# apple/ml-fastvlm

Hardware: AMD Instinct MI355X
Metric: images/sec FastViTHD encode_images @1024x1024 bf16 (higher is better)
Workload: dtype bf16; 1 GPU; BASELINE.json configs[1]: FastViTHD encoder + mlp2x_gelu projector (H=896), batch=32/GPU synthetic 1024x1024 bf16 images in [0,1), seeded synthetic weights, single GPU; global_batch=32, image_size=1024, parallelism=dp1, hip_graph=False, attention_operands=bf16, ffn_precision=auto (calibrated on the benchmark batch), range guard on

## Files before the change

### include/fvhd.h

```cpp
#ifndef FVHD_H
#define FVHD_H

#include <stddef.h>
#include <stdint.h>

#ifdef __cplusplus
extern "C" {
#endif

typedef struct fvhd_ctx fvhd_ctx;
typedef void* fvhd_stream_t;

#define FVHD_F32 0
#define FVHD_F16 1
#define FVHD_BF16 2

#define FVHD_EPI_NONE 0
#define FVHD_EPI_BIAS 1
#define FVHD_EPI_BIAS_GELU 2
#define FVHD_EPI_BIAS_LS_RESID 3

#define FVHD_VERSION 510
int fvhd_version(void);
const char* fvhd_last_error(void);
// ... 57 lines not shown
int fvhd_op_dw3_dw7(fvhd_stream_t stream, const void* x, void* y, void* a, const float* w3, const float* b3, const float* w7,
                    const float* b7, int B, int H, int W, int C, void* amax_bits);
int fvhd_dw3_dw7_supported(int B, int H, int W, int C, int force);
int fvhd_dw7s2_mfma_supported(int B, int H, int W, int Cin, int force);
int fvhd_op_dw7s2_mfma(fvhd_stream_t stream, const void* x, void* y, const float* w, const float* bias, int B, int H, int W, int Cin);
#define FVHD_AMAX_SLOTS 64
int fvhd_op_dw7_amax(fvhd_stream_t stream, const void* x, void* y, const float* w, const float* bias, int B, int H, int W, int C, int mfma,
                     void* amax_bits);
int fvhd_op_gemm(fvhd_stream_t stream, const void* A, const void* Wt, const float* bias, const float* ls,
                 const void* resid, void* out, int M, int N, int K, int epilogue, int out_dtype);
int fvhd_op_gemm_splitk_ls(fvhd_stream_t stream, const void* A, const void* Wt, const float* bias, const float* ls, const void* resid, void* out,
                           float* partial, int M, int N, int K, int splits);
int fvhd_gemm_splitk_plan(int M, int N, int K);
#define FVHD_GEMM_PLAN_V1_NF4_BK64 0
#define FVHD_GEMM_PLAN_V1_NF4_BK32 1
#define FVHD_GEMM_PLAN_V1_NF3_BK64 2
#define FVHD_GEMM_PLAN_V1_NF3_BK32 3
#define FVHD_GEMM_PLAN_V1S 4
#define FVHD_GEMM_PLAN_256X128 5
#define FVHD_GEMM_PLAN_256X256 6
#define FVHD_GEMM_PLAN_PINGPONG 7
#define FVHD_GEMM_PLAN_128X192 8
int fvhd_gemm_kernel_plan(int M, int N, int K, int epilogue, int out_dtype);
int fvhd_op_layernorm(fvhd_stream_t stream, const void* x, void* y, const float* w, const float* b, int M, int C, float eps);
int fvhd_op_attention(fvhd_stream_t stream, const void* qkv, void* out, int B, int N, int C);
int fvhd_op_attention_fp8(fvhd_stream_t stream, const void* qkv, void* out, int B, int N, int C);
int fvhd_op_stem_conv(fvhd_stream_t stream, const void* img, int dtype, void* out, const float* w, const float* bias, int B, int R);
int fvhd_op_stem_fused(fvhd_stream_t stream, const void* img, int dtype, void* out, const float* w0, const float* b0,
                       const float* w1, const float* b1, const void* w2, const float* b2, int B, int R);
int fvhd_op_se_head(fvhd_stream_t stream, const void* y, float* pooled, float* scale, const float* wr, const float* br,
                    const float* we, const float* be, void* out, int out_dtype, int B, int T, int C, int RD);

int fvhd_ffn_fused_supported(int C);
int fvhd_ffn_pack(int C, const float* host_fc1, const float* host_fc2, void* host_w1img, void* host_w2img, int precision);
int fvhd_op_ffn_fused(fvhd_stream_t stream, const void* A, const void* w1img, const float* b1, const void* w2img,
                      const float* b2, const float* ls, void* X, int M, int C, int precision);

int fvhd_op_preprocess(fvhd_stream_t stream, const void* src, int src_h, int src_w, int64_t src_pitch, int pad_top, int pad_left,
                       uint32_t bg, const int32_t* hbounds, const int32_t* hcoef, int hk, const int32_t* vbounds, const int32_t* vcoef,
                       int vk, int row0, int nrows, void* tmp, const float* lut, int R, void* out, int out_dtype);

int fvhd_op_splice(fvhd_stream_t stream, const int64_t* ids, const int32_t* start, const int32_t* seqlen, const int64_t* feat_row0,
                   const int64_t* labels_in, const void* table, const void* feats, void* out, uint8_t* mask_out, int64_t* pos_out,
                   int64_t* labels_out, int B, int L, int H, int max_len, int64_t vocab, int64_t n_feat_rows, int left_pad, int dtype);

#define FVHD_EPI_RESID 4
// ... 148 lines not shown
```

### ml_fastvlm_amd/_lib.py

```python
from __future__ import annotations

import ctypes as C
import os
from typing import Dict, Tuple

_HERE = os.path.dirname(os.path.abspath(__file__))
LIB_PATH = os.environ.get("FVHD_LIB") or os.path.join(_HERE, "libfvhd.so")

ABI_VERSION = 501
SAMPLING_VERSION = 502
WIDE_BATCH_VERSION = 503
W8_VERSION = 504
BEAM_VERSION = 505
PROCESSORS_VERSION = 506
LOOKUP_VERSION = 507
GEMM_PLAN_VERSION = 508
EXTEND_VERSION = 509
(GEMM_PLAN_V1_NF4_BK64, GEMM_PLAN_V1_NF4_BK32, GEMM_PLAN_V1_NF3_BK64, GEMM_PLAN_V1_NF3_BK32, GEMM_PLAN_V1S, GEMM_PLAN_256X128, GEMM_PLAN_256X256,
 GEMM_PLAN_PINGPONG, GEMM_PLAN_128X192) = range(9)
MAX_DECODE_BATCH = 64
MAX_VERIFY_ROWS = 16
MAX_EOS_IDS, MAX_SUPPRESS_IDS = 16, 256
MAX_LOGPROBS = 16
W_BF16, W_E4M3 = 0, 1
# ... 140 lines not shown
            "fvhd_llm_cache_rewind": (ci, [vp, vp, vp]),
            "fvhd_op_attention_extend": (ci, [vp, vp, vp, vp, vp, vp, ci, ci, ci, ci, ci, ci, vp]),
            "fvhd_op_cache_append": (ci, [vp, vp, vp, vp, vp, vp, ci, ci, ci, ci, ci, ci, vp, vp]),
            "fvhd_op_extend_positions": (ci, [vp, vp, vp, vp, ci, ci]),
            "fvhd_op_cache_rewind": (ci, [vp, vp, ci, vp, vp, ci, vp, vp]),
        })
    if hasattr(lib, "fvhd_op_lm_score"):
        sig.update({
            "fvhd_lm_score_scratch_bytes": (C.c_size_t, [ci, ci, ci]),
            "fvhd_lm_score_plan": (ci, [ci, ci, ci]),
            "fvhd_op_lm_score": (ci, [vp, vp, vp, vp, ci, ci, ci, vp, vp, vp, C.c_size_t]),
            "fvhd_llm_score_reserve": (ci, [vp, ci]),
            "fvhd_llm_score": (ci, [vp, vp, vp, vp, vp]),
        })
    if hasattr(lib, "fvhd_op_dec_gemm_w4"):
        sig.update({
            "fvhd_llm_debug_packed_mxfp4": (ci, [vp, ci, ci, vp, vp, vp]),
            "fvhd_op_quantize_mxfp4": (ci, [vp, vp, ci, ci, vp, vp]),
            "fvhd_op_dec_gemm_w4": (ci, [vp, ci, vp, ci, vp, cf, vp, vp, ci, ci, vp, vp, vp, vp, ci]),
            "fvhd_op_dec_qkv_w4": (ci, [vp, vp, ci, ci, vp, cf, vp, vp, vp, vp, vp, vp, ci, cf, vp, vp, ci, vp, ci, ci, ci, vp, vp, ci]),
            "fvhd_op_dec_lm_argmax_w4": (ci, [vp, vp, ci, vp, cf, vp, vp, ci, ci, vp, vp, vp, vp]),
            "fvhd_op_w4_unpack": (ci, [vp, vp, vp, vp, ci, ci, ci]),
        })
    if hasattr(lib, "fvhd_op_dec_logprobs"):
        sig.update({
            "fvhd_dec_logprobs_scratch_bytes": (C.c_size_t, [ci, ci, ci]),
            "fvhd_op_dec_logprobs": (ci, [vp, vp, vp, ci, ci, ci, vp, vp, vp, vp, C.c_size_t]),
            "fvhd_llm_set_logprobs": (ci, [vp, ci]),
            "fvhd_llm_logprobs": (ci, [vp, vp, ci, vp, vp, vp, vp]),
        })
    del fp, cl
    for name, (res, args) in sig.items():
        fn = getattr(lib, name)
        fn.restype = res
        fn.argtypes = args


def load():
    global _lib
    if _lib is None:
        if not os.path.exists(LIB_PATH):
            raise FvhdError(
                f"{LIB_PATH} not found: the HIP extension is not built. Run `python -m ml_fastvlm_amd.build` "
                "(hipcc, gfx950). There is no CPU fallback for this path.")
        lib = C.CDLL(LIB_PATH)
        lib.fvhd_version.restype, lib.fvhd_version.argtypes = C.c_int, []
# ... 37 lines not shown
    lib = load()
    got = lib.fvhd_version()
    if got < PROCESSORS_VERSION:
        raise FvhdError(f"{LIB_PATH} reports ABI version {got}: logits processors (fvhd_llm_set_logits_processors, "
                        f"fvhd_op_dec_logits_process) need {PROCESSORS_VERSION} - rebuild the library (`python -m ml_fastvlm_amd.build`)")
    return lib


def lookup_lib():
    lib = load()
    got = lib.fvhd_version()
    if got < LOOKUP_VERSION:
        raise FvhdError(f"{LIB_PATH} reports ABI version {got}: prompt-lookup decoding (fvhd_llm_spec_reserve, fvhd_llm_verify, "
                        f"fvhd_llm_lookup_step, ...) needs {LOOKUP_VERSION} - rebuild the library (`python -m ml_fastvlm_amd.build`)")
    return lib


def gemm_plan_lib():
    lib = load()
    got = lib.fvhd_version()
    if got < GEMM_PLAN_VERSION:
        raise FvhdError(f"{LIB_PATH} reports ABI version {got}: the GEMM dispatch query (fvhd_gemm_kernel_plan) needs {GEMM_PLAN_VERSION} - "
                        "rebuild the library (`python -m ml_fastvlm_amd.build`)")
    return lib


def extend_lib():
    lib = load()
    got = lib.fvhd_version()
    if got < EXTEND_VERSION:
        raise FvhdError(f"{LIB_PATH} reports ABI version {got}: extending a started cache (fvhd_llm_extend, fvhd_llm_cache_rewind, "
                        f"fvhd_op_attention_extend, ...) needs {EXTEND_VERSION} - rebuild the library (`python -m ml_fastvlm_amd.build`)")
    return lib


def score_lib():
    lib = load()
    if not hasattr(lib, "fvhd_op_lm_score"):
        raise FvhdError(f"{LIB_PATH} (ABI version {lib.fvhd_version()}) was built before scoring (fvhd_llm_score, fvhd_llm_score_reserve, "
                        "fvhd_op_lm_score, ...) - rebuild the library (`python -m ml_fastvlm_amd.build`)")
    return lib


def w4_lib():
    lib = load()
    if not hasattr(lib, "fvhd_op_dec_gemm_w4"):
# ... 201 lines not shown
```

### ml_fastvlm_amd/csrc/fvhd_api.hip

```cpp
#include <hip/hip_runtime.h>
#include <stdint.h>
#include <stdlib.h>
#include <string.h>

#include <cmath>
#include <map>
#include <string>
#include <vector>

#include "api_host.h"
#include "launchers.h"

namespace {

thread_local std::string g_err;

int fail(const std::string& msg, int code = 1)
{
    g_err = msg;
    return code ? code : 1;
}

int hip_fail(const char* what, hipError_t e)
{
// ... 1151 lines not shown
    }
    return e ? hip_fail("fvhd_op_dw7_amax", (hipError_t)e) : 0;
}

int fvhd_op_gemm(fvhd_stream_t st, const void* A, const void* Wt, const float* bias, const float* ls, const void* resid,
                 void* out, int M, int N, int K, int epilogue, int out_dtype)
{
    if (!A || !Wt || !out) return fail("fvhd_op_gemm: NULL pointer");
    if ((epilogue == FVHD_EPI_BIAS || epilogue == FVHD_EPI_BIAS_GELU || epilogue == FVHD_EPI_BIAS_LS_RESID) && !bias) return fail("fvhd_op_gemm: this epilogue needs bias");
    if (epilogue == FVHD_EPI_BIAS_LS_RESID && !ls) return fail("fvhd_op_gemm: FVHD_EPI_BIAS_LS_RESID needs ls");
    if ((epilogue == FVHD_EPI_BIAS_LS_RESID || epilogue == FVHD_EPI_RESID) && !resid) return fail("fvhd_op_gemm: this epilogue needs resid");
    int e = fvhd_launch_gemm((hipStream_t)st, A, Wt, bias, ls, resid, out, M, N, K, epilogue, out_dtype);
    return e ? hip_fail("fvhd_op_gemm", (hipError_t)e) : 0;
}

int fvhd_op_gemm_splitk_ls(fvhd_stream_t st, const void* A, const void* Wt, const float* bias, const float* ls, const void* resid, void* out,
                           float* partial, int M, int N, int K, int splits)
{
    if (!A || !Wt || !bias || !ls || !resid || !out || !partial) return fail("fvhd_op_gemm_splitk_ls: NULL pointer");
    int e = fvhd_launch_gemm_splitk_ls((hipStream_t)st, A, Wt, bias, ls, resid, out, partial, M, N, K, splits);
    return e ? hip_fail("fvhd_op_gemm_splitk_ls", (hipError_t)e) : 0;
}

int fvhd_op_layernorm(fvhd_stream_t st, const void* x, void* y, const float* w, const float* b, int M, int C, float eps)
{
    int e = fvhd_launch_layernorm((hipStream_t)st, x, y, w, b, M, C, eps);
    return e ? hip_fail("fvhd_op_layernorm", (hipError_t)e) : 0;
}

int fvhd_op_attention(fvhd_stream_t st, const void* qkv, void* out, int B, int N, int C)
{
    int e = fvhd_launch_attention((hipStream_t)st, qkv, out, B, N, C, 0);
    return e ? hip_fail("fvhd_op_attention", (hipError_t)e) : 0;
}

int fvhd_op_attention_fp8(fvhd_stream_t st, const void* qkv, void* out, int B, int N, int C)
{
    int e = fvhd_launch_attention((hipStream_t)st, qkv, out, B, N, C, 1);
    return e ? hip_fail("fvhd_op_attention_fp8", (hipError_t)e) : 0;
}

int fvhd_op_stem_conv(fvhd_stream_t st, const void* img, int dtype, void* out, const float* w, const float* bias, int B, int R)
{
    int e = fvhd_launch_stem_conv((hipStream_t)st, img, dtype, out, w, bias, B, R);
    return e ? hip_fail("fvhd_op_stem_conv", (hipError_t)e) : 0;
}
// ... 88 lines not shown
```

### ml_fastvlm_amd/csrc/gemm.hip

```cpp
#include "fvhd_common.h"
#include "launchers.h"
#include "gemm_layout.h"
#include "rope.h"
#include <stdlib.h>

#define EPI_NONE 0
#define EPI_BIAS 1
#define EPI_BIAS_GELU 2
#define EPI_BIAS_LS_RESID 3
#define EPI_RESID 4
static_assert(FVHD_EPI_SWIGLU_ID == 5 && FVHD_ODT_BF16_ID == FVHD_BF16, "gemm_layout.h ids");
#define EPI_SWIGLU 5

#define EPI_BIAS_ROPE 6

struct RopeArgs {
    const long* pos; const float* table; bf16* kcache; bf16* vcache;
    int M, T, nh, nkv, P; float theta;
};

template <int BK>
FVHD_DEV int lds_off(int row, int ks)
{
    if constexpr (BK == 64) return row * 128 + ((ks ^ ((row >> 1) & 7)) << 4);
// ... 222 lines not shown
#pragma unroll
            for (int i = 0; i < W_CH; ++i) rw[i] = *(const u32x4*)(w_src[i] + ko);
        }
#pragma unroll
        for (int kk = 0; kk < BK / 32; ++kk) {
            bf16x8 af[MF], wf[NF];
            const int ks = kk * 4 + g;
#pragma unroll
            for (int i = 0; i < MF; ++i) af[i] = *(const bf16x8*)(ldsA + lds_off<BK>(wm * 64 + i * 16 + lr, ks));
#pragma unroll
            for (int j = 0; j < NF; ++j) wf[j] = *(const bf16x8*)(ldsW + lds_off<BK>(wn * 16 * NF + j * 16 + lr, ks));
#pragma unroll
            for (int i = 0; i < MF; ++i)
#pragma unroll
                for (int j = 0; j < NF; ++j)
                    acc[i][j] = __builtin_amdgcn_mfma_f32_16x16x32_bf16(wf[j], af[i], acc[i][j], 0, 0, 0);
        }
    }

    gemm_epilogue<MF, NF, EPI, ODT>(acc, bias, ls, resid, out, M, N, m0 + wm * 64, n0 + wn * 16 * NF, lr, g);
}

template <int BN, int BK = 64, int NWV = 8> struct G2Cfg {
    static constexpr int RS = BK == 64 ? (BN == 256 ? 2 : 3) : (NWV == 4 ? 3 : BN == 256 ? 4 : 6), STAGE = (256 + BN) * BK * 2, LDS = RS * STAGE;
};
template <int BK> FVHD_DEV int lds_swz(int row) { return BK == 64 ? ((row >> 1) & 7) : ((0 - (row >> 2)) & 3); }

FVHD_DEV void glds_piece(unsigned voff, const void* sbase, unsigned m0v)
{
    unsigned keep;
    asm volatile("s_mov_b32 %0, m0\n\ts_mov_b32 m0, %3\n\ts_nop 0\n\tglobal_load_lds_dwordx4 %1, %2\n\ts_mov_b32 m0, %0"
                 : "=&s"(keep) : "v"(voff), "s"(sbase), "s"(m0v) : "memory");
}

template <int EPI, int ODT, int NWV, int BN = 128, int BKT = 64, int ABL = 0>
__global__ __launch_bounds__(64 * NWV, (NWV == 4 && BKT == 32) ? 2 : 1) void gemm256_kernel(
    const bf16* __restrict__ A, const bf16* __restrict__ Wt, const float* __restrict__ bias,
    const float* __restrict__ ls, const bf16* resid, void* out, int M, int N, int K, int tiles_n, int nwg)
{
    constexpr int BM = 256, BK = BKT, WN = BN / 64, WM = NWV / WN, MF = BM / WM / 16, NF = 4, RS = G2Cfg<BN, BK, NWV>::RS, STAGE = G2Cfg<BN, BK, NWV>::STAGE;
    constexpr int RPP = 1024 / (BK * 2), LPR = BK / 8;
    constexpr int PA = (BM / RPP) / NWV, PW = (BN / RPP) / NWV;
    static_assert(WM * WN == NWV && MF * 16 * WM == BM, "wave grid");
    extern __shared__ __attribute__((aligned(16))) char lds2[];
    const int tid = threadIdx.x, lane = tid & 63, wave = __builtin_amdgcn_readfirstlane(tid >> 6);
    const int wm = wave / WN, wn = wave % WN;
    const int lr = lane & 15, g = lane >> 4;
    constexpr int GN = BN == 256 ? 4 : 8;
    const int tiles_m = nwg / tiles_n;
    auto tile_origin = [&](int t, int& m0_, int& n0_) {
        const int L = xcd_remap(t, nwg);
        const int grp = L / (tiles_m * GN), rem = L - grp * tiles_m * GN;
        const int wg = min(GN, tiles_n - grp * GN);
        const int tm = rem / wg, tn = grp * GN + (rem - tm * wg);
        m0_ = tm * BM; n0_ = tn * BN;
    };
    int tile = blockIdx.x, m0, n0;
    tile_origin(tile, m0, n0);

    constexpr int GRP = EpiGrp<NF, EPI, ODT>::value;
    static_assert(GRP == 1 || BK == 64, "the W row permutation is written for 8-row pieces");
    const int rip = lane / LPR;
    unsigned va[2], vw[2];
#pragma unroll
    for (int par = 0; par < 2; ++par) {
        const int sw = lds_swz<BK>(par * RPP + rip);
        va[par] = (unsigned)((rip * K + (((lane % LPR) ^ sw) * 8)) * 2);
        vw[par] = (unsigned)((wpiece_lane_row<GRP>(rip) * K + (((lane % LPR) ^ sw) * 8)) * 2);
    }
    const char* abase = (const char*)(A + (size_t)(m0 + wave * RPP * PA) * K);
    const char* wbase = (const char*)(Wt + (size_t)n0 * K);
// ... 24 lines not shown
        for (int j = 0; j < NF; ++j) acc[i][j] = f32x4{0.f, 0.f, 0.f, 0.f};

    for (int kt = 0; kt < nk; ++kt) {
        {
            const int later = nk - 1 - kt < RS - 2 ? nk - 1 - kt : RS - 2;
            if (later == RS - 2 && RS > 2) asm volatile("s_waitcnt vmcnt(%0)" :: "n"((RS - 2) * (PA + PW)) : "memory");
            else if (RS > 5 && later == 3) asm volatile("s_waitcnt vmcnt(%0)" :: "n"(3 * (PA + PW)) : "memory");
            else if (RS > 4 && later == 2) asm volatile("s_waitcnt vmcnt(%0)" :: "n"(2 * (PA + PW)) : "memory");
            else if (RS > 3 && later == 1) asm volatile("s_waitcnt vmcnt(%0)" :: "n"(1 * (PA + PW)) : "memory");
            else asm volatile("s_waitcnt vmcnt(0)" ::: "memory");
        }
        __syncthreads();
        if (kt + RS - 1 < nk) issue(kt + RS - 1);
        const char* ldsA = lds2 + (kt % RS) * STAGE;
        const char* ldsW = ldsA + BM * BK * 2;
        if constexpr (ABL == 2) continue;
#pragma unroll
        for (int kk = 0; kk < BK / 32; ++kk) {
            bf16x8 af[MF], wf[NF];
            const int ks = kk * 4 + g;
#pragma unroll
            for (int i = 0; i < MF; ++i) af[i] = *(const bf16x8*)(ldsA + lds_off<BK>(wm * 16 * MF + i * 16 + lr, ks));
#pragma unroll
            for (int j = 0; j < NF; ++j) wf[j] = *(const bf16x8*)(ldsW + lds_off<BK>(wn * 64 + j * 16 + lr, ks));
#pragma unroll
            for (int i = 0; i < MF; ++i)
#pragma unroll
                for (int j = 0; j < NF; ++j)
                    acc[i][j] = __builtin_amdgcn_mfma_f32_16x16x32_bf16(wf[j], af[i], acc[i][j], 0, 0, 0);
        }
    }
    const int em0 = m0 + wm * 16 * MF, en0 = n0 + wn * 64;
    tile += gridDim.x;
    const bool more = tile < nwg;
    if (more) {
        __syncthreads();
        tile_origin(tile, m0, n0);
        abase = (const char*)(A + (size_t)(m0 + wave * RPP * PA) * K);
        wbase = (const char*)(Wt + (size_t)n0 * K);
#pragma unroll
        for (int i = 0; i < RS - 1; ++i)
            if (i < nk) issue(i);
    }
    gemm_epilogue<MF, NF, EPI, ODT, true>(acc, bias, ls, resid, out, M, N, em0, en0, lr, g);
    if (!more) break;
  }
}

constexpr int kG128Stages = 4, kG128Stage = (128 + 128) * 64 * 2, kG128Lds = kG128Stages * kG128Stage;
template <int EPI, int ODT>
__global__ __launch_bounds__(256, 1) void gemm128s_kernel(
    const bf16* __restrict__ A, const bf16* __restrict__ Wt, const float* __restrict__ bias,
    const float* __restrict__ ls, const bf16* resid, void* out_, int M, int N, int K, int tiles_n, int nwg, int ldk, RopeArgs rope)
{
    constexpr int BM = 128, BK = 64, MF = 4, NF = 4, RS = kG128Stages, STAGE = kG128Stage, RPP = 8, PA = 4, PW = 4;
// ... 54 lines not shown
        __syncthreads();
        if (kt + RS - 1 < nk) issue(kt + RS - 1);
        const char* ldsA = lds2 + (kt % RS) * STAGE;
        const char* ldsW = ldsA + BM * BK * 2;
#pragma unroll
        for (int kk = 0; kk < BK / 32; ++kk) {
            bf16x8 af[MF], wf[NF];
            const int ks = kk * 4 + g;
#pragma unroll
            for (int i = 0; i < MF; ++i) af[i] = *(const bf16x8*)(ldsA + lds_off<BK>(wm * 64 + i * 16 + lr, ks));
#pragma unroll
            for (int j = 0; j < NF; ++j) wf[j] = *(const bf16x8*)(ldsW + lds_off<BK>(wn * 64 + j * 16 + lr, ks));
#pragma unroll
            for (int i = 0; i < MF; ++i)
#pragma unroll
                for (int j = 0; j < NF; ++j)
                    acc[i][j] = __builtin_amdgcn_mfma_f32_16x16x32_bf16(wf[j], af[i], acc[i][j], 0, 0, 0);
        }
    }
    if constexpr (EPI == EPI_BIAS_ROPE) gemm_epilogue_rope<MF>(acc, bias, (bf16*)out, rope, M, N, m0 + wm * 64, n0 + wn * 64, lr, g);
    else gemm_epilogue<MF, NF, EPI, ODT, true>(acc, bias, ls, resid, out, M, N, m0 + wm * 64, n0 + wn * 64, lr, g);
}

template <int EPI, int ODT>
__global__ __launch_bounds__(512) void gemm_pp_kernel(
    const bf16* __restrict__ A, const bf16* __restrict__ Wt, const float* __restrict__ bias,
    const float* __restrict__ ls, const bf16* resid, void* out, int M, int N, int K, int tiles_n, int nwg)
{
    constexpr int BM = 256, BN = 256, BK = 64, MF = 8, NF = 4, STAGE = (BM + BN) * 128;
    extern __shared__ __attribute__((aligned(16))) char lds2[];
    const int tid = threadIdx.x, lane = tid & 63, wave = __builtin_amdgcn_readfirstlane(tid >> 6);
    const int grp = wave >> 2, wn = wave & 3;
    const int lr = lane & 15, g = lane >> 4;
    const int L = xcd_remap(blockIdx.x, nwg);
    constexpr int GN = 4;
    const int tiles_m = nwg / tiles_n;
    const int sg = L / (tiles_m * GN), rem = L - sg * tiles_m * GN;
    const int wgw = min(GN, tiles_n - sg * GN);
    const int tm = rem / wgw, tn = sg * GN + (rem - tm * wgw);
    const int m0 = tm * BM, n0 = tn * BN;

    constexpr int GRP = EpiGrp<NF, EPI, ODT>::value;
    const int rip = lane >> 3;
    unsigned vo[2], vwo[2];
#pragma unroll
    for (int par = 0; par < 2; ++par) {
        const int sw = ((par * 8 + rip) >> 1) & 7;
        vo[par] = (unsigned)((rip * K + (((lane & 7) ^ sw) * 8)) * 2);
        vwo[par] = (unsigned)((wpiece_lane_row<GRP>(rip) * K + (((lane & 7) ^ sw) * 8)) * 2);
    }
    const char* abase = (const char*)(A + (size_t)(m0 + wave * 32) * K);
    const char* wbase = (const char*)(Wt + (size_t)n0 * K);
    const unsigned lds0 = lds_addr(lds2);
    auto issue4 = [&](int kt, int which) {
        const unsigned st = lds0 + (kt & 1) * STAGE + (which ? 256 * 128 : 0) + wave * 4096;
        if (which) {
#pragma unroll
            for (int j = 0; j < 4; ++j)
                glds_piece(vwo[j & 1], wbase + (size_t)wpiece_row<GRP>(wave * 4 + j) * K * 2 + (size_t)kt * BK * 2, st + j * 1024);
        } else {
            const char* base = abase + (size_t)kt * BK * 2;
#pragma unroll
            for (int j = 0; j < 4; ++j) glds_piece(vo[j & 1], base + (size_t)j * 8 * K * 2, st + j * 1024);
        }
    };

    f32x4 acc[MF][NF];
#pragma unroll
    for (int i = 0; i < MF; ++i)
#pragma unroll
        for (int j = 0; j < NF; ++j) acc[i][j] = f32x4{0.f, 0.f, 0.f, 0.f};
    bf16x8 af[MF], wf[NF];

    const int nk = K / BK;
    issue4(0, 0); issue4(0, 1);
    if (nk > 1) { issue4(1, 0); issue4(1, 1); }
    asm volatile("s_waitcnt vmcnt(0)" ::: "memory");
    __builtin_amdgcn_s_barrier();
    if (grp == 1) __builtin_amdgcn_s_barrier();

    auto load_phase = [&](int kt, int h) {
        const char* ldsA = lds2 + (kt & 1) * STAGE;
        const char* ldsW = ldsA + 256 * 128;
        const int ks = h * 4 + g;
#pragma unroll
        for (int j = 0; j < NF; ++j) wf[j] = *(const bf16x8*)(ldsW + lds_off<BK>(wn * 64 + j * 16 + lr, ks));
#pragma unroll
        for (int i = 0; i < MF; ++i) af[i] = *(const bf16x8*)(ldsA + lds_off<BK>(grp * 128 + i * 16 + lr, ks));
    };
    auto mfma_phase = [&]() {
        __builtin_amdgcn_s_setprio(1);
#pragma unroll
        for (int i = 0; i < MF; ++i)
#pragma unroll
            for (int j = 0; j < NF; ++j)
                acc[i][j] = __builtin_amdgcn_mfma_f32_16x16x32_bf16(wf[j], af[i], acc[i][j], 0, 0, 0);
        __builtin_amdgcn_s_setprio(0);
    };
#define PP_END(WAIT_VM)                                                                           \
    do {                                                                                          \
        if (WAIT_VM) asm volatile("s_waitcnt vmcnt(0) lgkmcnt(0)" ::: "memory");                  \
        else asm volatile("s_waitcnt lgkmcnt(0)" ::: "memory");                                   \
        __builtin_amdgcn_s_barrier();                                                             \
        __builtin_amdgcn_sched_barrier(0);                                                        \
    } while (0)

    for (int kt = 0; kt < nk; ++kt) {
        const bool d1 = kt >= 1 && kt + 1 < nk, d2 = kt + 2 < nk;
        load_phase(kt, 0);
        if (d1) issue4(kt + 1, grp == 0 ? 0 : 1);
        PP_END(false);
        mfma_phase();
        if (d1 && grp == 0) issue4(kt + 1, 1);
        PP_END(false);
        load_phase(kt, 1);
        PP_END(grp == 1);
        mfma_phase();
        if (d2 && grp == 1) issue4(kt + 2, 0);
        PP_END(grp == 0);
    }
    if (grp == 0) __builtin_amdgcn_s_barrier();
#undef PP_END
    gemm_epilogue<MF, NF, EPI, ODT, true>(acc, bias, ls, resid, out, M, N, m0 + grp * 128, n0 + wn * 64, lr, g);
}

#ifndef FVHD_GEMM_PERSIST_DEFAULT
#define FVHD_GEMM_PERSIST_DEFAULT 0
#endif
static int cu_count()
{
    static int cached[64] = {};
    int dev = 0;
    (void)hipGetDevice(&dev);
    int& n = cached[dev & 63];
    if (n <= 0) {
        int v = 0;
        if (hipDeviceGetAttribute(&v, hipDeviceAttributeMultiprocessorCount, dev) != hipSuccess || v <= 0) v = 256;
        n = v;
    }
    return n;
}

#ifdef FVHD_DEBUG_KNOBS
static int g_gemm_v2 = 1;
extern "C" void fvhd_debug_set_gemm_v2(int on) { g_gemm_v2 = on; }
#else
// ... 5 lines not shown
static hipError_t launch_gemm256(hipStream_t st, const bf16* A, const bf16* Wt, const float* bias, const float* ls,
                                 const bf16* resid, void* out, int M, int N, int K)
{
    static bool attr_set[64] = {};
    int dev = 0;
    (void)hipGetDevice(&dev);
    if (!attr_set[dev & 63]) {
        hipError_t e = hipFuncSetAttribute((const void*)gemm256_kernel<EPI, ODT, NWV, BN, BKT, ABL>, hipFuncAttributeMaxDynamicSharedMemorySize, G2Cfg<BN, BKT, NWV>::LDS);
        if (e != hipSuccess) return e;
        attr_set[dev & 63] = true;
    }
    const int tiles_m = M / 256, tiles_n = N / BN, nwg = tiles_m * tiles_n;
    constexpr int LDSB = G2Cfg<BN, BKT, NWV>::LDS;
    static const int persist = [] { const char* ev = getenv("FVHD_GEMM_PERSIST"); return ev ? atoi(ev) : FVHD_GEMM_PERSIST_DEFAULT; }();
    int grid = nwg;
    if (persist && ABL == 0) {
        const int g8 = cu_count() & ~7;
        if (g8 >= 8 && nwg > g8) grid = g8;
    }
    hipLaunchKernelGGL((gemm256_kernel<EPI, ODT, NWV, BN, BKT, ABL>), dim3(grid), dim3(64 * NWV), LDSB, st, A, Wt, bias, ls, resid, out, M, N, K, tiles_n, nwg);
    return hipGetLastError();
}

template <int EPI, int ODT>
static hipError_t launch_gemm_pp(hipStream_t st, const bf16* A, const bf16* Wt, const float* bias, const float* ls,
                                 const bf16* resid, void* out, int M, int N, int K)
{
    constexpr int LDS = 2 * 512 * 128;
    static bool attr_set[64] = {};
    int dev = 0;
    (void)hipGetDevice(&dev);
    if (!attr_set[dev & 63]) {
        hipError_t e = hipFuncSetAttribute((const void*)gemm_pp_kernel<EPI, ODT>, hipFuncAttributeMaxDynamicSharedMemorySize, LDS);
        if (e != hipSuccess) return e;
        attr_set[dev & 63] = true;
    }
    const int tiles_m = M / 256, tiles_n = N / 256, nwg = tiles_m * tiles_n;
    hipLaunchKernelGGL((gemm_pp_kernel<EPI, ODT>), dim3(nwg), dim3(512), LDS, st, A, Wt, bias, ls, resid, out, M, N, K, tiles_n, nwg);
    return hipGetLastError();
}

static hipError_t dispatch_gemm_pp(hipStream_t st, const bf16* a, const bf16* w, const float* bias, const float* ls, const bf16* r, void* out,
                                   int M, int N, int K, int epi)
{
    switch (epi) {
    case EPI_NONE: return launch_gemm_pp<EPI_NONE, FVHD_BF16>(st, a, w, bias, ls, r, out, M, N, K);
    case EPI_BIAS: return launch_gemm_pp<EPI_BIAS, FVHD_BF16>(st, a, w, bias, ls, r, out, M, N, K);
    case EPI_BIAS_GELU: return launch_gemm_pp<EPI_BIAS_GELU, FVHD_BF16>(st, a, w, bias, ls, r, out, M, N, K);
    case EPI_BIAS_LS_RESID: return launch_gemm_pp<EPI_BIAS_LS_RESID, FVHD_BF16>(st, a, w, bias, ls, r, out, M, N, K);
    case EPI_RESID: return launch_gemm_pp<EPI_RESID, FVHD_BF16>(st, a, w, bias, ls, r, out, M, N, K);
    case EPI_SWIGLU: return launch_gemm_pp<EPI_SWIGLU, FVHD_BF16>(st, a, w, bias, ls, r, out, M, N, K);
    }
    return hipErrorInvalidValue;
}

template <int BN>
static hipError_t dispatch_gemm256(hipStream_t st, const bf16* a, const bf16* w, const float* bias, const float* ls, const bf16* r, void* out,
                                   int M, int N, int K, int epi)
{
    switch (epi) {
    case EPI_NONE: return launch_gemm256<EPI_NONE, FVHD_BF16, 8, BN>(st, a, w, bias, ls, r, out, M, N, K);
    case EPI_BIAS: return launch_gemm256<EPI_BIAS, FVHD_BF16, 8, BN>(st, a, w, bias, ls, r, out, M, N, K);
// ... 195 lines not shown
template <int NF, int BK>
static hipError_t dispatch_epi(hipStream_t st, const bf16* A, const bf16* Wt, const float* bias, const float* ls,
                               const bf16* resid, void* out, int M, int N, int K, int epi, int odt)
{
    if (odt == FVHD_BF16) {
        switch (epi) {
        case EPI_NONE: return launch_gemm<NF, BK, EPI_NONE, FVHD_BF16>(st, A, Wt, bias, ls, resid, out, M, N, K);
        case EPI_BIAS: return launch_gemm<NF, BK, EPI_BIAS, FVHD_BF16>(st, A, Wt, bias, ls, resid, out, M, N, K);
        case EPI_BIAS_GELU: return launch_gemm<NF, BK, EPI_BIAS_GELU, FVHD_BF16>(st, A, Wt, bias, ls, resid, out, M, N, K);
        case EPI_BIAS_LS_RESID: return launch_gemm<NF, BK, EPI_BIAS_LS_RESID, FVHD_BF16>(st, A, Wt, bias, ls, resid, out, M, N, K);
        case EPI_RESID: return launch_gemm<NF, BK, EPI_RESID, FVHD_BF16>(st, A, Wt, bias, ls, resid, out, M, N, K);
        case EPI_SWIGLU: return launch_gemm<NF, BK, EPI_SWIGLU, FVHD_BF16>(st, A, Wt, bias, ls, resid, out, M, N, K);
        }
    } else if (epi == EPI_BIAS) {
        if (odt == FVHD_F16) return launch_gemm<NF, BK, EPI_BIAS, FVHD_F16>(st, A, Wt, bias, ls, resid, out, M, N, K);
        if (odt == FVHD_F32) return launch_gemm<NF, BK, EPI_BIAS, FVHD_F32>(st, A, Wt, bias, ls, resid, out, M, N, K);
    } else if (epi == EPI_NONE && odt == FVHD_F32) {
        return launch_gemm<NF, BK, EPI_NONE, FVHD_F32>(st, A, Wt, bias, ls, resid, out, M, N, K);
    }
    return hipErrorInvalidValue;
}

constexpr int kPlanAblate = 100;
static int gemm_plan(int M, int N, int K, int epi, int out_dtype)
{
    if (M <= 0 || N <= 0 || K <= 0 || (K % 32) || (N % 16)) return -1;
    if (out_dtype == FVHD_BF16 ? (epi < EPI_NONE || epi > EPI_SWIGLU)
                               : !((epi == EPI_BIAS && (out_dtype == FVHD_F16 || out_dtype == FVHD_F32)) || (epi == EPI_NONE && out_dtype == FVHD_F32)))
        return -1;
    if (out_dtype == FVHD_BF16 && take_gemm128s(M, N, K, (long)(M / 128) * (N / 128))) return FVHD_GEMM_PLAN_V1S;
    if (g_gemm_v2 && out_dtype == FVHD_BF16 && M % 256 == 0 && N % 128 == 0 && K % 64 == 0 && K >= 128) {
        const long long t128 = (long long)(M / 256) * (N / 128), t256 = N % 256 == 0 ? (long long)(M / 256) * (N / 256) : 0;
#ifdef FVHD_DEBUG_KNOBS
        if ((g_gemm_v2 == 8 || g_gemm_v2 == 9) && t256 > 0 && (epi == EPI_NONE || epi == EPI_BIAS_GELU)) return kPlanAblate;
#endif
        const long long ncu = cu_count();
        const bool use256 = g_gemm_v2 == 3 ? t256 > 0 : (g_gemm_v2 == 1 && N >= 2304 && t256 * 4 >= ncu * 7);
        const long long rounds128 = (t128 + ncu - 1) / ncu;
        const bool full_enough = t128 >= 4 * ncu || t128 * 5 >= rounds128 * ncu * 4;
        const bool use128 = g_gemm_v2 == 2 || (g_gemm_v2 == 1 && ((t128 >= 2 * ncu && full_enough) || (t128 * 2 >= ncu && K >= 3072)));
        if ((g_gemm_v2 == 4 && t256 > 0) || (g_gemm_v2 == 1 && K >= 3072 && t256 * 2 >= ncu)) return FVHD_GEMM_PLAN_PINGPONG;
        if (use256) return FVHD_GEMM_PLAN_256X256;
        if (use128) return FVHD_GEMM_PLAN_256X128;
    }
    const bool nf3 = (N % 128 != 0) && (N % 96 == 0);
    const bool bk64 = (K % 64 == 0);
    if (g_gemm_nf6 && nf3 && bk64 && N % 192 == 0 && epi == EPI_BIAS_GELU && out_dtype == FVHD_BF16 && (long long)((M + 127) / 128) * (N / 192) >= 4ll * cu_count())
        return FVHD_GEMM_PLAN_128X192;
    if (nf3) return bk64 ? FVHD_GEMM_PLAN_V1_NF3_BK64 : FVHD_GEMM_PLAN_V1_NF3_BK32;
    return bk64 ? FVHD_GEMM_PLAN_V1_NF4_BK64 : FVHD_GEMM_PLAN_V1_NF4_BK32;
}

extern "C" int fvhd_gemm_kernel_plan(int M, int N, int K, int epilogue, int out_dtype)
{
    const int p = gemm_plan(M, N, K, epilogue, out_dtype);
    return p == kPlanAblate ? -1 : p;
}

extern "C" int fvhd_launch_gemm(hipStream_t st, const void* A, const void* Wt, const float* bias, const float* ls,
                                const void* resid, void* out, int M, int N, int K, int epi, int out_dtype)
{
    const bf16* a = (const bf16*)A;
    const bf16* w = (const bf16*)Wt;
    const bf16* r = (const bf16*)resid;
    const bool reads_bias = epi == EPI_BIAS || epi == EPI_BIAS_GELU || epi == EPI_BIAS_LS_RESID, reads_resid = epi == EPI_BIAS_LS_RESID || epi == EPI_RESID;
    if (!A || !Wt || !out || (reads_bias && !bias) || (epi == EPI_BIAS_LS_RESID && !ls) || (reads_resid && !resid)) return (int)hipErrorInvalidValue;
    switch (gemm_plan(M, N, K, epi, out_dtype)) {
    case FVHD_GEMM_PLAN_V1S: return (int)dispatch_gemm128s(st, a, w, bias, ls, r, out, M, N, K, epi);
    case FVHD_GEMM_PLAN_PINGPONG: return (int)dispatch_gemm_pp(st, a, w, bias, ls, r, out, M, N, K, epi);
    case FVHD_GEMM_PLAN_256X256: return (int)dispatch_gemm256<256>(st, a, w, bias, ls, r, out, M, N, K, epi);
    case FVHD_GEMM_PLAN_256X128: return (int)dispatch_gemm256<128>(st, a, w, bias, ls, r, out, M, N, K, epi);
    case FVHD_GEMM_PLAN_128X192: return (int)launch_gemm<6, 64, EPI_BIAS_GELU, FVHD_BF16>(st, a, w, bias, ls, r, out, M, N, K);
    case FVHD_GEMM_PLAN_V1_NF3_BK64: return (int)dispatch_epi<3, 64>(st, a, w, bias, ls, r, out, M, N, K, epi, out_dtype);
    case FVHD_GEMM_PLAN_V1_NF3_BK32: return (int)dispatch_epi<3, 32>(st, a, w, bias, ls, r, out, M, N, K, epi, out_dtype);
    case FVHD_GEMM_PLAN_V1_NF4_BK64: return (int)dispatch_epi<4, 64>(st, a, w, bias, ls, r, out, M, N, K, epi, out_dtype);
    case FVHD_GEMM_PLAN_V1_NF4_BK32: return (int)dispatch_epi<4, 32>(st, a, w, bias, ls, r, out, M, N, K, epi, out_dtype);
#ifdef FVHD_DEBUG_KNOBS
    case kPlanAblate:
        if (g_gemm_v2 == 8) return (int)(epi == EPI_NONE ? launch_gemm256<EPI_NONE, FVHD_BF16, 8, 256, 64, 1>(st, a, w, bias, ls, r, out, M, N, K)
                                                          : launch_gemm256<EPI_BIAS_GELU, FVHD_BF16, 8, 256, 64, 1>(st, a, w, bias, ls, r, out, M, N, K));
        return (int)(epi == EPI_NONE ? launch_gemm256<EPI_NONE, FVHD_BF16, 8, 256, 64, 2>(st, a, w, bias, ls, r, out, M, N, K)
                                     : launch_gemm256<EPI_BIAS_GELU, FVHD_BF16, 8, 256, 64, 2>(st, a, w, bias, ls, r, out, M, N, K));
#endif
    }
    return (int)hipErrorInvalidValue;
}
```

### ml_fastvlm_amd/csrc/launchers.h

```cpp
#pragma once
#include <hip/hip_runtime.h>
#include "../../include/fvhd.h"
#include "llm_decode.h"

extern "C" {
int fvhd_set_error(const char* msg);
int fvhd_launch_dwconv(hipStream_t st, const void* x, void* y, const float* w, const float* bias, int B, int H, int W, int Cin, int K, int stride, int mult, int gelu,
                       int flags, unsigned* amax);
int fvhd_dw7_mfma_supported(int B, int H, int W, int C, int force);
int fvhd_launch_dw7_mfma(hipStream_t st, const void* x, void* y, const float* w, const float* bias, int B, int H, int W, int C, unsigned* amax);
int fvhd_launch_dw7s2_mfma(hipStream_t st, const void* x, void* y, const float* w, const float* bias, int B, int H, int W, int Cin, int gelu);
int fvhd_launch_dw3_dw7(hipStream_t st, const void* x, void* y, void* a, const float* w3, const float* b3, const float* w7, const float* b7, int B, int H, int W, int C,
                        unsigned* amax);
int fvhd_launch_gemm(hipStream_t st, const void* A, const void* Wt, const float* bias, const float* ls, const void* resid, void* out, int M, int N, int K, int epi,
                     int out_dtype);
int fvhd_launch_gemm_splitk(hipStream_t st, const void* A, const void* Wt, const void* resid, void* out, float* partial, int M, int N, int K, int splits);
int fvhd_launch_gemm_splitk_ls(hipStream_t st, const void* A, const void* Wt, const float* bias, const float* ls, const void* resid, void* out, float* partial, int M,
                               int N, int K, int splits);
int fvhd_launch_gemm_splitk_partials(hipStream_t st, const void* A, const void* Wt, float* partial, int M, int N, int K, int splits);
int fvhd_launch_gemm_splitk_norm(hipStream_t st, const void* A, const void* Wt, const void* resid, void* out, float* partial, int M, int N, int K, int splits,
                                 const float* norm_w, void* norm_out, float eps);
int fvhd_launch_gemm_qkv_rope(hipStream_t st, const void* A, const void* Wt, const float* bias, void* out, int Mp, int N, int K, const long* pos, const float* table,
                              void* kcache, void* vcache, int M, int T, int nh, int nkv, int HD, int P, float theta);
int fvhd_launch_layernorm(hipStream_t st, const void* x, void* y, const float* w, const float* b, int M, int C, float eps);
int fvhd_launch_attention(hipStream_t st, const void* qkv, void* out, int B, int N, int C, int fp8);
int fvhd_launch_stem_conv(hipStream_t st, const void* img, int dtype, void* out, const float* w, const float* bias, int B, int R);
int fvhd_launch_stem_fused(hipStream_t st, const void* img, int dtype, void* out, const float* w0, const float* b0, const float* w1, const float* b1, const void* w2,
                           const float* b2, int B, int R);
int fvhd_launch_se_head(hipStream_t st, const void* y, float* pooled, float* scale, const float* wr, const float* br, const float* we, const float* be, void* out,
                        int out_dtype, int B, int T, int C, int RD);
int fvhd_launch_cast_to_bf16(hipStream_t st, const void* x, int dtype, void* y, long n);
int fvhd_ffn_pack_host(int C, const float* fc1, const float* fc2, uint16_t* w1img, uint16_t* w2img, int precision);
float fvhd_ffn_half_w2_limit(void);
int fvhd_launch_ffn_fused(hipStream_t st, const void* A, const void* w1img, const float* b1, const void* w2img, const float* b2, const float* ls, void* X, int M, int C,
                          int precision);
int fvhd_launch_splice(hipStream_t st, const long* ids, const int* start, const int* seqlen, const long* feat_row0, const long* labels_in, const void* table,
                       const void* feats, void* out, unsigned char* mask_out, long* pos_out, long* labels_out, int B, int L, int H, int max_len, long vocab,
                       long n_feat_rows, int left_pad, int dtype);
// ... 59 lines not shown
```

Measured before the change: 1497 images/sec.

## Add 256x192 GEMM tiles for streaming and ping-pong kernels with wave-quantization dispatch

Result: no change. 1499 images/sec, median of 4 (+0.1%).

```diff
diff --git a/include/fvhd.h b/include/fvhd.h
--- a/include/fvhd.h
+++ b/include/fvhd.h
@@ -103,6 +103,9 @@
 #define FVHD_GEMM_PLAN_PINGPONG 7
 #define FVHD_GEMM_PLAN_128X192 8
 int fvhd_gemm_kernel_plan(int M, int N, int K, int epilogue, int out_dtype);
+int fvhd_gemm_tile_n(int M, int N, int K, int epilogue, int out_dtype);
+int fvhd_op_gemm_bn192(fvhd_stream_t stream, const void* A, const void* Wt, const float* bias, const float* ls, const void* resid, void* out,
+                       int M, int N, int K, int epilogue, int out_dtype, int family);
 int fvhd_op_layernorm(fvhd_stream_t stream, const void* x, void* y, const float* w, const float* b, int M, int C, float eps);
 int fvhd_op_attention(fvhd_stream_t stream, const void* qkv, void* out, int B, int N, int C);
 int fvhd_op_attention_fp8(fvhd_stream_t stream, const void* qkv, void* out, int B, int N, int C);
diff --git a/ml_fastvlm_amd/_lib.py b/ml_fastvlm_amd/_lib.py
--- a/ml_fastvlm_amd/_lib.py
+++ b/ml_fastvlm_amd/_lib.py
@@ -186,6 +186,11 @@
             "fvhd_op_dec_lm_argmax_w4": (ci, [vp, vp, ci, vp, cf, vp, vp, ci, ci, vp, vp, vp, vp]),
             "fvhd_op_w4_unpack": (ci, [vp, vp, vp, vp, ci, ci, ci]),
         })
+    if hasattr(lib, "fvhd_op_gemm_bn192"):
+        sig.update({
+            "fvhd_gemm_tile_n": (ci, [ci, ci, ci, ci, ci]),
+            "fvhd_op_gemm_bn192": (ci, [vp, vp, vp, vp, vp, vp, vp, ci, ci, ci, ci, ci, ci]),
+        })
     if hasattr(lib, "fvhd_op_dec_logprobs"):
         sig.update({
             "fvhd_dec_logprobs_scratch_bytes": (C.c_size_t, [ci, ci, ci]),
@@ -269,6 +274,14 @@
     if got < GEMM_PLAN_VERSION:
         raise FvhdError(f"{LIB_PATH} reports ABI version {got}: the GEMM dispatch query (fvhd_gemm_kernel_plan) needs {GEMM_PLAN_VERSION} - "
                         "rebuild the library (`python -m ml_fastvlm_amd.build`)")
+    return lib
+
+
+def gemm_bn192_lib():
+    lib = load()
+    if not hasattr(lib, "fvhd_op_gemm_bn192"):
+        raise FvhdError(f"{LIB_PATH} (ABI version {lib.fvhd_version()}) was built before the 256 x 192 GEMM tiles (fvhd_gemm_tile_n, "
+                        "fvhd_op_gemm_bn192) - rebuild the library (`python -m ml_fastvlm_amd.build`)")
     return lib
 
 
diff --git a/ml_fastvlm_amd/csrc/fvhd_api.hip b/ml_fastvlm_amd/csrc/fvhd_api.hip
--- a/ml_fastvlm_amd/csrc/fvhd_api.hip
+++ b/ml_fastvlm_amd/csrc/fvhd_api.hip
@@ -1197,6 +1197,20 @@
     return e ? hip_fail("fvhd_op_gemm_splitk_ls", (hipError_t)e) : 0;
 }
 
+int fvhd_op_gemm_bn192(fvhd_stream_t st, const void* A, const void* Wt, const float* bias, const float* ls, const void* resid, void* out,
+                       int M, int N, int K, int epilogue, int out_dtype, int family)
+{
+    if (!A || !Wt || !out) return fail("fvhd_op_gemm_bn192: NULL pointer");
+    if (out_dtype != FVHD_BF16) return fail("fvhd_op_gemm_bn192: the output must be bf16");
+    if (family != 0 && family != 1) return fail("fvhd_op_gemm_bn192: family must be 0 (streaming) or 1 (ping-pong)");
+    if (epilogue < FVHD_EPI_NONE || epilogue > FVHD_EPI_BIAS_LS_RESID) return fail("fvhd_op_gemm_bn192: epilogue must be NONE, BIAS, BIAS_GELU or BIAS_LS_RESID");
+    if (epilogue != FVHD_EPI_NONE && !bias) return fail("fvhd_op_gemm_bn192: this epilogue needs bias");
+    if (epilogue == FVHD_EPI_BIAS_LS_RESID && (!ls || !resid)) return fail("fvhd_op_gemm_bn192: FVHD_EPI_BIAS_LS_RESID needs ls and resid");
+    if (M <= 0 || N <= 0 || M % 256 || N % 192 || K % 64 || K < 128) return fail("fvhd_op_gemm_bn192: needs M % 256 == 0, N % 192 == 0, K % 64 == 0, K >= 128");
+    int e = fvhd_launch_gemm_bn192((hipStream_t)st, A, Wt, bias, ls, resid, out, M, N, K, epilogue, family);
+    return e ? hip_fail("fvhd_op_gemm_bn192", (hipError_t)e) : 0;
+}
+
 int fvhd_op_layernorm(fvhd_stream_t st, const void* x, void* y, const float* w, const float* b, int M, int C, float eps)
 {
     int e = fvhd_launch_layernorm((hipStream_t)st, x, y, w, b, M, C, eps);
diff --git a/ml_fastvlm_amd/csrc/gemm.hip b/ml_fastvlm_amd/csrc/gemm.hip
--- a/ml_fastvlm_amd/csrc/gemm.hip
+++ b/ml_fastvlm_amd/csrc/gemm.hip
@@ -268,7 +268,7 @@
 }
 
 template <int BN, int BK = 64, int NWV = 8> struct G2Cfg {
-    static constexpr int RS = BK == 64 ? (BN == 256 ? 2 : 3) : (NWV == 4 ? 3 : BN == 256 ? 4 : 6), STAGE = (256 + BN) * BK * 2, LDS = RS * STAGE;
+    static constexpr int RS = BK == 64 ? (BN >= 192 ? 2 : 3) : (NWV == 4 ? 3 : BN == 256 ? 4 : 6), STAGE = (256 + BN) * BK * 2, LDS = RS * STAGE;
 };
 template <int BK> FVHD_DEV int lds_swz(int row) { return BK == 64 ? ((row >> 1) & 7) : ((0 - (row >> 2)) & 3); }
 
@@ -284,15 +284,15 @@
     const bf16* __restrict__ A, const bf16* __restrict__ Wt, const float* __restrict__ bias,
     const float* __restrict__ ls, const bf16* resid, void* out, int M, int N, int K, int tiles_n, int nwg)
 {
-    constexpr int BM = 256, BK = BKT, WN = BN / 64, WM = NWV / WN, MF = BM / WM / 16, NF = 4, RS = G2Cfg<BN, BK, NWV>::RS, STAGE = G2Cfg<BN, BK, NWV>::STAGE;
+    constexpr int BM = 256, BK = BKT, WN = BN == 192 ? 4 : BN / 64, WM = NWV / WN, MF = BM / WM / 16, NF = BN / WN / 16, RS = G2Cfg<BN, BK, NWV>::RS, STAGE = G2Cfg<BN, BK, NWV>::STAGE;
     constexpr int RPP = 1024 / (BK * 2), LPR = BK / 8;
     constexpr int PA = (BM / RPP) / NWV, PW = (BN / RPP) / NWV;
-    static_assert(WM * WN == NWV && MF * 16 * WM == BM, "wave grid");
+    static_assert(WM * WN == NWV && MF * 16 * WM == BM && NF * 16 * WN == BN && PW * NWV * RPP == BN && PA * NWV * RPP == BM, "wave grid");
     extern __shared__ __attribute__((aligned(16))) char lds2[];
     const int tid = threadIdx.x, lane = tid & 63, wave = __builtin_amdgcn_readfirstlane(tid >> 6);
     const int wm = wave / WN, wn = wave % WN;
     const int lr = lane & 15, g = lane >> 4;
-    constexpr int GN = BN == 256 ? 4 : 8;
+    constexpr int GN = BN >= 192 ? 4 : 8;
     const int tiles_m = nwg / tiles_n;
     auto tile_origin = [&](int t, int& m0_, int& n0_) {
         const int L = xcd_remap(t, nwg);
@@ -363,7 +363,7 @@
 #pragma unroll
             for (int i = 0; i < MF; ++i) af[i] = *(const bf16x8*)(ldsA + lds_off<BK>(wm * 16 * MF + i * 16 + lr, ks));
 #pragma unroll
-            for (int j = 0; j < NF; ++j) wf[j] = *(const bf16x8*)(ldsW + lds_off<BK>(wn * 64 + j * 16 + lr, ks));
+            for (int j = 0; j < NF; ++j) wf[j] = *(const bf16x8*)(ldsW + lds_off<BK>(wn * 16 * NF + j * 16 + lr, ks));
 #pragma unroll
             for (int i = 0; i < MF; ++i)
 #pragma unroll
@@ -371,7 +371,7 @@
                     acc[i][j] = __builtin_amdgcn_mfma_f32_16x16x32_bf16(wf[j], af[i], acc[i][j], 0, 0, 0);
         }
     }
-    const int em0 = m0 + wm * 16 * MF, en0 = n0 + wn * 64;
+    const int em0 = m0 + wm * 16 * MF, en0 = n0 + wn * 16 * NF;
     tile += gridDim.x;
     const bool more = tile < nwg;
     if (more) {
@@ -472,12 +472,13 @@
     else gemm_epilogue<MF, NF, EPI, ODT, true>(acc, bias, ls, resid, out, M, N, m0 + wm * 64, n0 + wn * 64, lr, g);
 }
 
-template <int EPI, int ODT>
+template <int EPI, int ODT, int BN = 256>
 __global__ __launch_bounds__(512) void gemm_pp_kernel(
     const bf16* __restrict__ A, const bf16* __restrict__ Wt, const float* __restrict__ bias,
     const float* __restrict__ ls, const bf16* resid, void* out, int M, int N, int K, int tiles_n, int nwg)
 {
-    constexpr int BM = 256, BN = 256, BK = 64, MF = 8, NF = 4, STAGE = (BM + BN) * 128;
+    constexpr int BM = 256, BK = 64, MF = 8, NF = BN / 64, PW = BN / 64, STAGE = (BM + BN) * 128;
+    static_assert(BN == 256 || BN == 192, "four waves side by side in N: 64 or 48 columns each");
     extern __shared__ __attribute__((aligned(16))) char lds2[];
     const int tid = threadIdx.x, lane = tid & 63, wave = __builtin_amdgcn_readfirstlane(tid >> 6);
     const int grp = wave >> 2, wn = wave & 3;
@@ -503,11 +504,14 @@
     const char* wbase = (const char*)(Wt + (size_t)n0 * K);
     const unsigned lds0 = lds_addr(lds2);
     auto issue4 = [&](int kt, int which) {
-        const unsigned st = lds0 + (kt & 1) * STAGE + (which ? 256 * 128 : 0) + wave * 4096;
+        const unsigned st = lds0 + (kt & 1) * STAGE + (which ? 256 * 128 + wave * PW * 1024 : wave * 4096);
         if (which) {
 #pragma unroll
-            for (int j = 0; j < 4; ++j)
-                glds_piece(vwo[j & 1], wbase + (size_t)wpiece_row<GRP>(wave * 4 + j) * K * 2 + (size_t)kt * BK * 2, st + j * 1024);
+            for (int j = 0; j < PW; ++j) {
+                const int pi = wave * PW + j;
+                const int wr = GRP == 1 ? pi * 8 : wpiece_row<GRP>(pi);
+                glds_piece(vwo[pi & 1], wbase + (size_t)wr * K * 2 + (size_t)kt * BK * 2, st + j * 1024);
+            }
         } else {
             const char* base = abase + (size_t)kt * BK * 2;
 #pragma unroll
@@ -534,7 +538,7 @@
         const char* ldsW = ldsA + 256 * 128;
         const int ks = h * 4 + g;
 #pragma unroll
-        for (int j = 0; j < NF; ++j) wf[j] = *(const bf16x8*)(ldsW + lds_off<BK>(wn * 64 + j * 16 + lr, ks));
+        for (int j = 0; j < NF; ++j) wf[j] = *(const bf16x8*)(ldsW + lds_off<BK>(wn * 16 * NF + j * 16 + lr, ks));
 #pragma unroll
         for (int i = 0; i < MF; ++i) af[i] = *(const bf16x8*)(ldsA + lds_off<BK>(grp * 128 + i * 16 + lr, ks));
     };
@@ -571,7 +575,7 @@
     }
     if (grp == 0) __builtin_amdgcn_s_barrier();
 #undef PP_END
-    gemm_epilogue<MF, NF, EPI, ODT, true>(acc, bias, ls, resid, out, M, N, m0 + grp * 128, n0 + wn * 64, lr, g);
+    gemm_epilogue<MF, NF, EPI, ODT, true>(acc, bias, ls, resid, out, M, N, m0 + grp * 128, n0 + wn * 16 * NF, lr, g);
 }
 
 #ifndef FVHD_GEMM_PERSIST_DEFAULT
@@ -623,22 +627,40 @@
     return hipGetLastError();
 }
 
-template <int EPI, int ODT>
+template <int EPI, int ODT, int BN = 256>
 static hipError_t launch_gemm_pp(hipStream_t st, const bf16* A, const bf16* Wt, const float* bias, const float* ls,
                                  const bf16* resid, void* out, int M, int N, int K)
 {
-    constexpr int LDS = 2 * 512 * 128;
+    constexpr int LDS = 2 * (256 + BN) * 128;
     static bool attr_set[64] = {};
     int dev = 0;
     (void)hipGetDevice(&dev);
     if (!attr_set[dev & 63]) {
-        hipError_t e = hipFuncSetAttribute((const void*)gemm_pp_kernel<EPI, ODT>, hipFuncAttributeMaxDynamicSharedMemorySize, LDS);
+        hipError_t e = hipFuncSetAttribute((const void*)gemm_pp_kernel<EPI, ODT, BN>, hipFuncAttributeMaxDynamicSharedMemorySize, LDS);
         if (e != hipSuccess) return e;
         attr_set[dev & 63] = true;
     }
-    const int tiles_m = M / 256, tiles_n = N / 256, nwg = tiles_m * tiles_n;
-    hipLaunchKernelGGL((gemm_pp_kernel<EPI, ODT>), dim3(nwg), dim3(512), LDS, st, A, Wt, bias, ls, resid, out, M, N, K, tiles_n, nwg);
+    const int tiles_m = M / 256, tiles_n = N / BN, nwg = tiles_m * tiles_n;
+    hipLaunchKernelGGL((gemm_pp_kernel<EPI, ODT, BN>), dim3(nwg), dim3(512), LDS, st, A, Wt, bias, ls, resid, out, M, N, K, tiles_n, nwg);
     return hipGetLastError();
+}
+
+template <bool PINGPONG>
+static hipError_t dispatch_gemm_bn192(hipStream_t st, const bf16* a, const bf16* w, const float* bias, const float* ls, const bf16* r, void* out,
+                                      int M, int N, int K, int epi)
+{
+#define FVHD_BN192_CASE(E)                                                                                             \
+    case E:                                                                                                            \
+        if constexpr (PINGPONG) return launch_gemm_pp<E, FVHD_BF16, 192>(st, a, w, bias, ls, r, out, M, N, K);         \
+        else return launch_gemm256<E, FVHD_BF16, 8, 192>(st, a, w, bias, ls, r, out, M, N, K)
+    switch (epi) {
+    FVHD_BN192_CASE(EPI_NONE);
+    FVHD_BN192_CASE(EPI_BIAS);
+    FVHD_BN192_CASE(EPI_BIAS_GELU);
+    FVHD_BN192_CASE(EPI_BIAS_LS_RESID);
+    }
+#undef FVHD_BN192_CASE
+    return hipErrorInvalidValue;
 }
 
 static hipError_t dispatch_gemm_pp(hipStream_t st, const bf16* a, const bf16* w, const float* bias, const float* ls, const bf16* r, void* out,
@@ -880,8 +902,17 @@
 }
 
 constexpr int kPlanAblate = 100;
-static int gemm_plan(int M, int N, int K, int epi, int out_dtype)
-{
+static const int g_gemm_bn192 = [] { const char* e = getenv("FVHD_GEMM_BN192"); return e ? atoi(e) : 1; }();
+static bool bn192_legal(int M, int N, int K, int epi, int out_dtype)
+{
+    return M > 0 && N > 0 && M % 256 == 0 && N % 192 == 0 && K % 64 == 0 && K >= 128 && epi >= EPI_NONE && epi <= EPI_BIAS_LS_RESID && out_dtype == FVHD_BF16;
+}
+constexpr int kBn192CostStreaming = 937, kBn192CostPingPong = 979;
+static int gemm_plan(int M, int N, int K, int epi, int out_dtype, int* tile_n = nullptr)
+{
+    int width_unused = 0;
+    int& width = tile_n ? *tile_n : width_unused;
+    width = 0;
     if (M <= 0 || N <= 0 || K <= 0 || (K % 32) || (N % 16)) return -1;
     if (out_dtype == FVHD_BF16 ? (epi < EPI_NONE || epi > EPI_SWIGLU)
                                : !((epi == EPI_BIAS && (out_dtype == FVHD_F16 || out_dtype == FVHD_F32)) || (epi == EPI_NONE && out_dtype == FVHD_F32)))
@@ -897,9 +928,12 @@
         const long long rounds128 = (t128 + ncu - 1) / ncu;
         const bool full_enough = t128 >= 4 * ncu || t128 * 5 >= rounds128 * ncu * 4;
         const bool use128 = g_gemm_v2 == 2 || (g_gemm_v2 == 1 && ((t128 >= 2 * ncu && full_enough) || (t128 * 2 >= ncu && K >= 3072)));
-        if ((g_gemm_v2 == 4 && t256 > 0) || (g_gemm_v2 == 1 && K >= 3072 && t256 * 2 >= ncu)) return FVHD_GEMM_PLAN_PINGPONG;
-        if (use256) return FVHD_GEMM_PLAN_256X256;
-        if (use128) return FVHD_GEMM_PLAN_256X128;
+        const long long t192 = g_gemm_bn192 && g_gemm_v2 == 1 && t256 > ncu && bn192_legal(M, N, K, epi, out_dtype) ? (long long)(M / 256) * (N / 192) : 0;
+        auto rounds = [&](long long t) { return (t + ncu - 1) / ncu; };
+        auto width_for = [&](int cost192) { return t192 > 0 && rounds(t192) * cost192 < rounds(t256) * 1000 ? 192 : 256; };
+        if ((g_gemm_v2 == 4 && t256 > 0) || (g_gemm_v2 == 1 && K >= 3072 && t256 * 2 >= ncu)) { width = width_for(kBn192CostPingPong); return FVHD_GEMM_PLAN_PINGPONG; }
+        if (use256) { width = width_for(kBn192CostStreaming); return FVHD_GEMM_PLAN_256X256; }
+        if (use128) { width = 128; return FVHD_GEMM_PLAN_256X128; }
     }
     const bool nf3 = (N % 128 != 0) && (N % 96 == 0);
     const bool bk64 = (K % 64 == 0);
@@ -915,6 +949,23 @@
     return p == kPlanAblate ? -1 : p;
 }
 
+extern "C" int fvhd_gemm_tile_n(int M, int N, int K, int epilogue, int out_dtype)
+{
+    int bn = 0;
+    const int p = gemm_plan(M, N, K, epilogue, out_dtype, &bn);
+    return p < 0 || p == kPlanAblate ? 0 : bn;
+}
+
+extern "C" int fvhd_launch_gemm_bn192(hipStream_t st, const void* A, const void* Wt, const float* bias, const float* ls, const void* resid, void* out,
+                                      int M, int N, int K, int epi, int family)
+{
+    const bool reads_bias = epi == EPI_BIAS || epi == EPI_BIAS_GELU || epi == EPI_BIAS_LS_RESID;
+    if (!A || !Wt || !out || (reads_bias && !bias) || (epi == EPI_BIAS_LS_RESID && (!ls || !resid))) return (int)hipErrorInvalidValue;
+    if (!bn192_legal(M, N, K, epi, FVHD_BF16) || (family != 0 && family != 1)) return (int)hipErrorInvalidValue;
+    return (int)(family ? dispatch_gemm_bn192<true>(st, (const bf16*)A, (const bf16*)Wt, bias, ls, (const bf16*)resid, out, M, N, K, epi)
+                        : dispatch_gemm_bn192<false>(st, (const bf16*)A, (const bf16*)Wt, bias, ls, (const bf16*)resid, out, M, N, K, epi));
+}
+
 extern "C" int fvhd_launch_gemm(hipStream_t st, const void* A, const void* Wt, const float* bias, const float* ls,
                                 const void* resid, void* out, int M, int N, int K, int epi, int out_dtype)
 {
@@ -923,10 +974,11 @@
     const bf16* r = (const bf16*)resid;
     const bool reads_bias = epi == EPI_BIAS || epi == EPI_BIAS_GELU || epi == EPI_BIAS_LS_RESID, reads_resid = epi == EPI_BIAS_LS_RESID || epi == EPI_RESID;
     if (!A || !Wt || !out || (reads_bias && !bias) || (epi == EPI_BIAS_LS_RESID && !ls) || (reads_resid && !resid)) return (int)hipErrorInvalidValue;
-    switch (gemm_plan(M, N, K, epi, out_dtype)) {
+    int bn = 0;
+    switch (gemm_plan(M, N, K, epi, out_dtype, &bn)) {
     case FVHD_GEMM_PLAN_V1S: return (int)dispatch_gemm128s(st, a, w, bias, ls, r, out, M, N, K, epi);
-    case FVHD_GEMM_PLAN_PINGPONG: return (int)dispatch_gemm_pp(st, a, w, bias, ls, r, out, M, N, K, epi);
-    case FVHD_GEMM_PLAN_256X256: return (int)dispatch_gemm256<256>(st, a, w, bias, ls, r, out, M, N, K, epi);
+    case FVHD_GEMM_PLAN_PINGPONG: return (int)(bn == 192 ? dispatch_gemm_bn192<true>(st, a, w, bias, ls, r, out, M, N, K, epi) : dispatch_gemm_pp(st, a, w, bias, ls, r, out, M, N, K, epi));
+    case FVHD_GEMM_PLAN_256X256: return (int)(bn == 192 ? dispatch_gemm_bn192<false>(st, a, w, bias, ls, r, out, M, N, K, epi) : dispatch_gemm256<256>(st, a, w, bias, ls, r, out, M, N, K, epi));
     case FVHD_GEMM_PLAN_256X128: return (int)dispatch_gemm256<128>(st, a, w, bias, ls, r, out, M, N, K, epi);
     case FVHD_GEMM_PLAN_128X192: return (int)launch_gemm<6, 64, EPI_BIAS_GELU, FVHD_BF16>(st, a, w, bias, ls, r, out, M, N, K);
     case FVHD_GEMM_PLAN_V1_NF3_BK64: return (int)dispatch_epi<3, 64>(st, a, w, bias, ls, r, out, M, N, K, epi, out_dtype);
diff --git a/ml_fastvlm_amd/csrc/launchers.h b/ml_fastvlm_amd/csrc/launchers.h
--- a/ml_fastvlm_amd/csrc/launchers.h
+++ b/ml_fastvlm_amd/csrc/launchers.h
@@ -14,6 +14,8 @@
                         unsigned* amax);
 int fvhd_launch_gemm(hipStream_t st, const void* A, const void* Wt, const float* bias, const float* ls, const void* resid, void* out, int M, int N, int K, int epi,
                      int out_dtype);
+int fvhd_launch_gemm_bn192(hipStream_t st, const void* A, const void* Wt, const float* bias, const float* ls, const void* resid, void* out, int M, int N, int K, int epi,
+                           int family);
 int fvhd_launch_gemm_splitk(hipStream_t st, const void* A, const void* Wt, const void* resid, void* out, float* partial, int M, int N, int K, int splits);
 int fvhd_launch_gemm_splitk_ls(hipStream_t st, const void* A, const void* Wt, const float* bias, const float* ls, const void* resid, void* out, float* partial, int M,
                                int N, int K, int splits);
```
